# CyberAgentAILab/layout-dm

Measured on AMD Instinct MI355X. Metric: layouts/sec (whole node), Rico25 uncond T=100, higher is better.
Workload: dtype f16 (f32 accumulate); 1 GPU; BASELINE config 2: rico25 cond=unconditional T=100 batch=512/GPU sampling=random; precision_mode=fast, launch=one launch per sampling call (reverse loop resident in the layout's workgroup), chunk_layouts=256, lanes=2, parallelism=dp1 (independent layout shards, one all_gather of the final tokens)

## Files before the change

layout_dm_amd/csrc/kernels_stack.hip:

```cpp
#include <cstdlib>

#include "ldm_kernels.h"
#include "ldm_dma.h"
#include "ldm_pipes.h"
#include "ldm_post_dpp.h"
#include "ldm_relation_core.h"

namespace ldm {

struct StackArgs {
  FusedLayerSet ls;
  float* x;
  int ldx, N, S, H, n_chunks;
  float scale_log2e;
  const char* head_img;
  const float *head_g, *head_b;
  float* logits;
  int ldl, n_head_tiles;
  PostArgs post;
  const float* adaln;
  StackTables tbl;
  int32_t* inter;
  int n_steps, inter_ld, tie_ld;
  int16_t t_model[kStackLoopMaxSteps], t_post[kStackLoopMaxSteps];
// ... 2 lines not shown
};
typedef const __attribute__((address_space(4))) StackArgs* stack_kargs_ptr;
__device__ __forceinline__ stack_kargs_ptr stack_kargs() {
  stack_kargs_ptr q = (stack_kargs_ptr)__builtin_amdgcn_kernarg_segment_ptr();
  asm volatile("" : "+s"(q));
  return q;
}
constexpr int kPostLd = 161;
constexpr int kPostRows = 128 * kPostLd * 4;
constexpr int kStackLoopB1 = 2048;
constexpr int kStackLoopRelLds = REL_MAX_EDGE * 4 + 4 * 32 * 4 + 16;
constexpr int kStackLoopLds = 1024 + 128 + 2304;
static_assert(kRelIncBytes <= 2304, "incidence lists outgrow their LDS slot");
static_assert(kRelScratchFloats * 4 <= 2 * KV_BYTES, "the SGD's scratch lives in the K / V buffers");

__device__ unsigned long long g_stack_phase[16];

__device__ __forceinline__ int stack_lane_id() {
  int l;
  asm volatile("v_mbcnt_lo_u32_b32 %0, -1, 0\n\tv_mbcnt_hi_u32_b32 %0, -1, %0" : "=v"(l));
  return l;
}

__device__ __forceinline__ float stack_xor32_swap(float v) {
  const auto sw = __builtin_amdgcn_permlane32_swap(__float_as_uint(v), __float_as_uint(v), false, false);
  return (stack_lane_id() & 32) ? __uint_as_float(sw[0]) : __uint_as_float(sw[1]);
}
#define LDM_XOR32(v) (HEAD == 2 ? stack_xor32_swap(v) : __shfl_xor(v, 32, 64))

template <bool TM, int HEAD, bool REL = false>
__global__ __launch_bounds__(256, 1) void stack_stream_k(StackArgs a) {
  static_assert(!REL || HEAD == 2, "the relation tail belongs to the loop kernel");
  constexpr int KS = 29, STAGE = TILE_STAGE, NT2 = 15, NGV = 58;
  extern __shared__ __attribute__((aligned(16))) char smem[];
  const int tid_o = threadIdx.x;
  const int wave_o = __builtin_amdgcn_readfirstlane(tid_o >> 6);
  const int b_o = blockIdx.x;

  unsigned long long t0 = 0, t_real0 = 0, s_pro = 0, s_stream = 0, s_core = 0, s_slab = 0, s_ln2 = 0, s_ffn = 0, s_bnd = 0, s_bnd_a = 0, s_bnd_b = 0, s_hsync = 0, s_ssync = 0;
  if constexpr (TM) {
    t0 = __builtin_amdgcn_s_memtime();
    t_real0 = __builtin_amdgcn_s_memrealtime();
  }
  f32x16 acc[NT2];
  if constexpr (HEAD == 2) {
    const stack_kargs_ptr kp = stack_kargs();
    const int S = kp->S;
    int* toks = reinterpret_cast<int*>(smem + 3 * STAGE + 2 * KV_BYTES + (3 * kp->H * 64 + 2 * LN_DP + 512 + kStackLoopB1 + 2 * LN_DP + 512) * 4);
    if (tid_o < 128) {
      const int s = tid_o < S ? tid_o : S - 1;
      const size_t row = (size_t)b_o * S + s;
      toks[tid_o] = kp->post.tokens[row];
      int cc = -1;
      if (kp->post.cond_seq) cc = kp->post.cond_seq[row] | ((kp->post.strong && kp->post.strong[row]) ? (1 << 30) : 0);
      toks[128 + tid_o] = cc;
    }
    if constexpr (REL) {
      if (tid_o == 0) {
        int k = 1;
        const int A5 = kp->post.v.n_attr;
        for (int e = 0; e < S / A5; ++e)
          toks[256 + e] = ((kp->post.cond_seq[(size_t)b_o * S + e * A5]) != kp->post.v.pad_id) ? k++ : -1;
      }
      const int e0 = kp->rel.edge_off[b_o], ne = kp->rel.edge_off[b_o + 1] - e0;
      relation_incidence(kp->rel, e0, ne, tid_o, S / kp->post.v.n_attr, reinterpret_cast<float*>(smem + 3 * STAGE), toks + 288,
                         reinterpret_cast<unsigned short*>(toks + 288 + kRelIncOffInts), [] { __syncthreads(); });
// ... 61 lines not shown
      v2[k] = in ? w.b2[i] : 0.f;
    }
    __builtin_amdgcn_sched_barrier(0);
#pragma unroll
    for (int k = 0; k < 6; ++k) sbias[tid + 256 * k] = vb[k];
#pragma unroll
    for (int k = 0; k < 8; ++k)
      if (tid + 256 * k < A.n_chunks * 32) sb1[tid + 256 * k] = v1[k];
#pragma unroll
    for (int k = 0; k < 2; ++k) {
      const int i = tid + 256 * k;
      sp[i] = 1.0f + vs[k];
      sp[LN_DP + i] = vh[k];
      sbo[i] = vo[k] + vh[k];
      sp2[i] = vg[k];
      sp2[LN_DP + i] = ve[k];
      sb2[i] = v2[k];
    }
  };
  auto dma_table = [&](const float* g, const float* lds_dst, int n_kib) {
    const unsigned dst = lds0 + (unsigned)(reinterpret_cast<const char*>(lds_dst) - smem);
    for (int k = wave; k < n_kib; k += 4) {
      asm volatile("s_mov_b32 m0, %0\n\ts_nop 0" ::"s"(dst + k * 1024) : "memory");
      dma_lin<0>(voff, reinterpret_cast<const char*>(g) + (size_t)k * 1024);
    }
  };
  auto dma_first_tiles = [&](const char* img) {
#pragma unroll
    for (int k = 0; k < 4; ++k) dma_lin4(voff, img + wave * 8192 + (k >> 1) * STAGE + (k & 1) * 4096,
                                         lds0 + wave * 8192 + (k >> 1) * STAGE + (k & 1) * 4096);
  };
  int t_model = 0;
  if constexpr (HEAD == 2) t_model = stack_kargs()->t_model[it];
#pragma unroll
  for (int i = 8; i < 16; ++i) acc[NT2 - 1][i] = to_agpr(0.f);
  if constexpr (HEAD == 2) {
    const int lane = stack_lane_id();
    const int r = lane & 31, hi = lane >> 5;
    const int row = wave * 32 + r;
    const int srow = row < S ? row : S - 1;
    const stack_kargs_ptr kp = stack_kargs();
    dma_table(kp->tbl.att_static, sbias, kStackTblAttStatic / 256);
    dma_table(kp->tbl.att_dyn + (size_t)t_model * L * kStackTblAttDyn, sp, kStackTblAttDyn / 256);
    const float* erow = kp->post.emb + (size_t)toks[srow] * kp->post.D + hi * 4;
    const float* prow = kp->post.pos + (size_t)srow * kp->post.D + hi * 4;
    constexpr int GB = 12;
#pragma unroll
    for (int g0 = 0; g0 < NGV; g0 += GB) {
      float4 re[GB], rp[GB];
#pragma unroll
      for (int i = 0; i < GB; ++i)
        if (g0 + i < NGV) {
          re[i] = *reinterpret_cast<const float4*>(erow + (g0 + i) * 8);
          rp[i] = *reinterpret_cast<const float4*>(prow + (g0 + i) * 8);
        }
      __builtin_amdgcn_sched_barrier(0);
#pragma unroll
      for (int i = 0; i < GB; ++i) {
        const int gg = g0 + i;
        if (gg < NGV) {
          const int t = gg >> 2, q0 = (gg & 3) * 4;
          acc[t][q0 + 0] = to_agpr(re[i].x + rp[i].x);
          acc[t][q0 + 1] = to_agpr(re[i].y + rp[i].y);
          acc[t][q0 + 2] = to_agpr(re[i].z + rp[i].z);
          acc[t][q0 + 3] = to_agpr(re[i].w + rp[i].w);
        }
      }
      __builtin_amdgcn_sched_barrier(0);
    }
  } else {
    const int lane = stack_lane_id();
    const int r = lane & 31, hi = lane >> 5;
    const int row = wave * 32 + r;
    const size_t m = (size_t)b * S + (row < S ? row : S - 1);
    constexpr int GB = 20;
    const float* rrow = A.x + m * A.ldx + hi * 4;
#pragma unroll
    for (int g0 = 0; g0 < NGV; g0 += GB) {
      float4 raw[GB];
#pragma unroll
      for (int i = 0; i < GB; ++i)
        if (g0 + i < NGV) raw[i] = *reinterpret_cast<const float4*>(rrow + (g0 + i) * 8);
      __builtin_amdgcn_sched_barrier(0);
#pragma unroll
      for (int i = 0; i < GB; ++i) {
        const int gg = g0 + i;
        if (gg < NGV) {
          const int t = gg >> 2, q0 = (gg & 3) * 4;
          acc[t][q0 + 0] = to_agpr(raw[i].x);
          acc[t][q0 + 1] = to_agpr(raw[i].y);
          acc[t][q0 + 2] = to_agpr(raw[i].z);
          acc[t][q0 + 3] = to_agpr(raw[i].w);
        }
      }
      __builtin_amdgcn_sched_barrier(0);
    }
  }
  if constexpr (TM) s_pro = __builtin_amdgcn_s_memtime() - t0;

  for (int l = 0; l < L; ++l) {
    const auto& w = A.ls.w[l];
    unsigned long long tL = 0;
    if constexpr (TM) tL = __builtin_amdgcn_s_memtime();
    f16x8 xf[KS];
    {
      if constexpr (HEAD == 2) {
        asm volatile("s_waitcnt vmcnt(0)" ::: "memory");
        __builtin_amdgcn_s_barrier();
        asm volatile("" ::: "memory");
        dma_first_tiles((const char*)w.img);
        dma_table(stack_kargs()->tbl.ffn + (size_t)l * kStackTblFfn, sb1, kStackTblFfn / 256);
      } else {
        __builtin_amdgcn_s_barrier();
        asm volatile("" ::: "memory");
        dma_first_tiles((const char*)w.img);
        stage_tables(w, w.ada_scale, w.ada_shift, tid);
        __syncthreads();
      }
      unsigned long long tE1 = 0, tE2 = 0;
      if constexpr (TM) tE1 = __builtin_amdgcn_s_memtime();
      const int lane3 = stack_lane_id();
      const int hi3 = lane3 >> 5;
      float s1 = 0.f, s2 = 0.f;
#pragma unroll
      for (int t = 0; t < NT2; ++t) {
        const f32x16 tile = acc[t];
#pragma unroll
        for (int i = 0; i < 16; ++i)
          if (t * 4 + (i >> 2) < NGV) {
            s1 += tile[i];
            s2 += tile[i] * tile[i];
          }
        __builtin_amdgcn_sched_barrier(0);
      }
      s1 += LDM_XOR32(s1);
      s2 += LDM_XOR32(s2);
      if constexpr (TM) tE2 = __builtin_amdgcn_s_memtime();
      constexpr float kInvN3 = 1.0f / 464.0f;
      const float mean = s1 * kInvN3;
      const float rstd = 1.0f / sqrtf(fmaxf(s2 * kInvN3 - mean * mean, 0.f) + 1e-5f);
      const float ra = rstd, rb = -mean * rstd;
      const float* gmp = sp + hi3 * 4;
      const float* tbp = sbo + hi3 * 4;
#pragma unroll
      for (int t = 0; t < NT2; ++t) {
        f32x16 tile = acc[t];
#pragma unroll
        for (int g = 0; g < 4; ++g) {
          const int gg = t * 4 + g;
// ... 76 lines not shown
          AC.hi = hi;
          AC.run(nf);
        }
        if constexpr (TM) tC = __builtin_amdgcn_s_memtime();
        {
          const int lane = stack_lane_id();
          const int r = lane & 31, hi = lane >> 5;
          SlabPair<NT2, TM> SP;
          SP.acc = acc;
          SP.voff = voff;
          SP.lds_w = lds0 + wave * 8192;
          SP.aS[0] = lds0 + r * 64 + (((0 + hi) ^ ((r >> 2) & 3)) << 4);
          SP.aS[1] = lds0 + r * 64 + (((2 + hi) ^ ((r >> 2) & 3)) << 4);
          SP.nf = nf;
          SP.gnext = gimg + (size_t)8 * STAGE;
          SP.run();
          if constexpr (TM) s_ssync += SP.t_sync;
        }
        if constexpr (TM) {
          s_stream += tB - tA;
          s_core += tC - tB;
          s_slab += __builtin_amdgcn_s_memtime() - tC;
        }
      }
    }
    unsigned long long t_att = 0, t_ln2 = 0;
    if constexpr (TM) t_att = __builtin_amdgcn_s_memtime();
    asm volatile("s_waitcnt vmcnt(0) lgkmcnt(0)" ::: "memory");
    __builtin_amdgcn_s_barrier();
    asm volatile("" ::: "memory");
    {
      const char* g0 = (const char*)w.ffn_img + wave * 16384;
#pragma unroll
      for (int k = 0; k < 4; ++k) dma_lin4(voff, g0 + k * 4096, lds0 + wave * 16384 + k * 4096);
    }
    if constexpr (HEAD == 2) {
      const stack_kargs_ptr kp = stack_kargs();
      if (l + 1 < L) {
        dma_table(kp->tbl.att_static + (size_t)(l + 1) * kStackTblAttStatic, sbias, kStackTblAttStatic / 256);
        dma_table(kp->tbl.att_dyn + ((size_t)t_model * L + l + 1) * kStackTblAttDyn, sp, kStackTblAttDyn / 256);
      } else {
        dma_table(kp->tbl.head, sp, kStackTblAttDyn / 256);
      }
    }
    const int lane2 = stack_lane_id();
    const int r2 = lane2 & 31, hi2 = lane2 >> 5;
    f16x8 xf2[KS];
    {
      float s1 = 0.f, s2 = 0.f;
#pragma unroll
      for (int t = 0; t < NT2; ++t) {
        const f32x16 tile = acc[t];
#pragma unroll
        for (int i = 0; i < 16; ++i)
          if (t * 4 + (i >> 2) < NGV) {
            s1 += tile[i];
            s2 += tile[i] * tile[i];
          }
        __builtin_amdgcn_sched_barrier(0);
      }
      s1 += LDM_XOR32(s1);
      s2 += LDM_XOR32(s2);
      constexpr float kInvN = 1.0f / 464.0f;
      const float mean = s1 * kInvN;
      const float rstd = 1.0f / sqrtf(fmaxf(s2 * kInvN - mean * mean, 0.f) + 1e-5f);
      const float* gp = sp2 + hi2 * 4;
      const float* bp = sb2 + hi2 * 4;
#pragma unroll
      for (int t = 0; t < NT2; ++t) {
        f32x16 tile = acc[t];
#pragma unroll
        for (int g = 0; g < 4; ++g) {
          const int gg = t * 4 + g;
          if (gg < NGV) {
            const int ks = gg >> 1, e0 = (gg & 1) * 4;
            const float4 ga = *reinterpret_cast<const float4*>(gp + gg * 8);
            const float4 be = *reinterpret_cast<const float4*>(gp + LN_DP + gg * 8);
            const float4 bb = *reinterpret_cast<const float4*>(bp + gg * 8);
            const float v0 = tile[g * 4 + 0], v1 = tile[g * 4 + 1], v2 = tile[g * 4 + 2], v3 = tile[g * 4 + 3];
            xf2[ks][e0 + 0] = (_Float16)fmaf((v0 - mean) * rstd, ga.x, be.x);
            xf2[ks][e0 + 1] = (_Float16)fmaf((v1 - mean) * rstd, ga.y, be.y);
            xf2[ks][e0 + 2] = (_Float16)fmaf((v2 - mean) * rstd, ga.z, be.z);
            xf2[ks][e0 + 3] = (_Float16)fmaf((v3 - mean) * rstd, ga.w, be.w);
            tile[g * 4 + 0] = v0 + bb.x;
            tile[g * 4 + 1] = v1 + bb.y;
            tile[g * 4 + 2] = v2 + bb.z;
            tile[g * 4 + 3] = v3 + bb.w;
            if (gg & 1) asm volatile("" : "+v"(xf2[ks]));
          }
        }
        asm volatile("" : "+a"(tile));
        acc[t] = tile;
        __builtin_amdgcn_sched_barrier(0);
      }
    }
    if constexpr (TM) t_ln2 = __builtin_amdgcn_s_memtime();
    {
      unsigned relW1[8], relW2[2];
#pragma unroll
      for (int k = 0; k < 8; ++k) relW1[k] = r2 * RKB + ((((k << 1) | hi2) ^ (r2 & 15)) << 4);
#pragma unroll
      for (int sx = 0; sx < 2; ++sx) relW2[sx] = r2 * 64 + (((2 * sx + hi2) ^ ((r2 >> 2) & 3)) << 4);
      const unsigned relB = lds0 + (unsigned)(reinterpret_cast<char*>(sb1) - smem) + hi2 * 16;
      FfnStream<KS, NT2, 2, false, 6, true> F;
      F.xf = xf2;
      F.acc = acc;
      F.voff = voff;
      asm volatile("s_waitcnt vmcnt(0) lgkmcnt(0)" ::: "memory");
      __builtin_amdgcn_s_barrier();
      asm volatile("" ::: "memory");
#pragma unroll
      for (int k = 0; k < 8; ++k) F.aW1[k] = lds0 + relW1[k];
#pragma unroll
      for (int sx = 0; sx < 2; ++sx) F.aW2[sx] = lds0 + relW2[sx];
      F.ab_next = relB;
#pragma unroll
      for (int k = 0; k < KS; ++k) asm volatile("" : "+v"(xf2[k]));
      __builtin_amdgcn_s_waitcnt(0x0F70);
      __builtin_amdgcn_sched_barrier(0);
      F.read_bias();
      F.template prologue<0>();
      {
        const f16x8 z = {(_Float16)0.f, (_Float16)0.f, (_Float16)0.f, (_Float16)0.f,
                         (_Float16)0.f, (_Float16)0.f, (_Float16)0.f, (_Float16)0.f};
        F.pf[0] = F.pf[1] = F.pfn[0] = F.pfn[1] = z;
      }
      const char* fimg = (const char*)w.ffn_img;
      for (int c = 0; c <= A.n_chunks; ++c) {
#if !defined(LDM_ABL_FFN_WINDOW)
        F.gnext = fimg + (size_t)(c == A.n_chunks ? 0 : c + 1) * FFN_STAGE + wave * 16384;
#elif LDM_ABL_FFN_WINDOW == 1
        F.gnext = fimg + wave * 16384;
#else
        F.gnext = fimg;
#endif
        F.mnext = lds0 + ((c + 1) & 1) * FFN_STAGE + wave * 16384;
        F.ab_next = relB + (c + 1 >= A.n_chunks ? 0 : c + 1) * 128;
        F.template step<0, true>();
      }
      asm volatile("s_waitcnt vmcnt(0) lgkmcnt(0)" ::: "memory");
      __builtin_amdgcn_sched_barrier(0);
    }
    unsigned long long t_ffn = 0;
    if constexpr (TM) {
      t_ffn = __builtin_amdgcn_s_memtime();
      s_ln2 += t_ln2 - t_att;
      s_ffn += t_ffn - t_ln2;
    }
  }
  if constexpr (TM) t_epi = __builtin_amdgcn_s_memtime();
  {
    __builtin_amdgcn_s_barrier();
    asm volatile("" ::: "memory");
    auto dma_head_tile = [&](int ht) {
      const char* g = A.head_img + (size_t)ht * STAGE + wave * 8192;
      const unsigned l = lds0 + (unsigned)(ht & 3) * STAGE + wave * 8192;
      dma_lin4(voff, g, l);
      dma_lin4(voff, g + 4096, l + 4096);
    };
    for (int ht = 0; ht < 3 && ht < A.n_head_tiles; ++ht) dma_head_tile(ht);
    if constexpr (HEAD != 2) {
      for (int i = tid_now(); i < LN_DP; i += 256) {
        sp[i] = i < A.N ? A.head_g[i] : 0.f;
        sp[LN_DP + i] = i < A.N ? A.head_b[i] : 0.f;
      }
    }
    __syncthreads();
    const int lane3 = stack_lane_id();
    const int r3 = lane3 & 31, hi3 = lane3 >> 5;
    const int row3 = wave * 32 + r3;
    f16x8 xf3[KS];
// ... 18 lines not shown
      const float ra = rstd, rb = -mean * rstd;
      const float* gmp = sp + hi3 * 4;
#pragma unroll
      for (int t = 0; t < NT2; ++t) {
        const f32x16 tile = acc[t];
#pragma unroll
        for (int g = 0; g < 4; ++g) {
          const int gg = t * 4 + g;
          if (gg < NGV) {
            const int ks = gg >> 1, e0 = (gg & 1) * 4;
            const float4 gm = *reinterpret_cast<const float4*>(gmp + gg * 8);
            const float4 be = *reinterpret_cast<const float4*>(gmp + LN_DP + gg * 8);
            xf3[ks][e0 + 0] = (_Float16)fmaf(fmaf(tile[g * 4 + 0], ra, rb), gm.x, be.x);
            xf3[ks][e0 + 1] = (_Float16)fmaf(fmaf(tile[g * 4 + 1], ra, rb), gm.y, be.y);
            xf3[ks][e0 + 2] = (_Float16)fmaf(fmaf(tile[g * 4 + 2], ra, rb), gm.z, be.z);
            xf3[ks][e0 + 3] = (_Float16)fmaf(fmaf(tile[g * 4 + 3], ra, rb), gm.w, be.w);
            if (gg & 1) asm volatile("" : "+v"(xf3[ks]));
          }
        }
        __builtin_amdgcn_sched_barrier(0);
      }
    }
#pragma unroll
    for (int k = 0; k < KS; ++k) asm volatile("" : "+v"(xf3[k]));
    __builtin_amdgcn_s_waitcnt(0x0F70);
    __builtin_amdgcn_sched_barrier(0);
    const bool valid3 = row3 < S;
    float* lrow = HEAD == 2 ? nullptr : A.logits + ((size_t)b * S + (valid3 ? row3 : S - 1)) * A.ldl + hi3 * 4;
    unsigned relW[8];
#pragma unroll
    for (int k = 0; k < 8; ++k) relW[k] = lds0 + r3 * RKB + ((((k << 1) | hi3) ^ (r3 & 15)) << 4);
    if constexpr (HEAD == 2) {
      constexpr int NHT = 5;
#pragma unroll
      for (int ht = 0; ht < NHT; ++ht) {
        asm volatile("s_waitcnt vmcnt(0) lgkmcnt(0)" ::: "memory");
        __builtin_amdgcn_s_barrier();
        asm volatile("" ::: "memory");
        if (ht + 3 < NHT) dma_head_tile(ht + 3);
        TilePipe<KS, 8> TP;
        TP.xf = xf3;
        TP.voff = voff;
#pragma unroll
        for (int k = 0; k < 8; ++k) TP.aW[k] = relW[k] + (unsigned)(ht & 3) * STAGE;
        TP.template run<false, false>();
        f32x16 lg = TP.acc;
        asm volatile("s_nop 7\n\ts_nop 7" : "+v"(lg));
        asm volatile("" : "+a"(lg));
        acc[ht] = lg;
      }
      __builtin_amdgcn_s_barrier();
      asm volatile("" ::: "memory");
      const stack_kargs_ptr kp = stack_kargs();
      const auto& p = kp->post;
      float* lgs = reinterpret_cast<float*>(smem);
      float4* rstat = reinterpret_cast<float4*>(smem + kPostRows);
      float* ssch = reinterpret_cast<float*>(smem + kPostRows + 2048) + wave * 128;
      const int Cm1 = p.v.n_class - 1;
      const int t_post = kp->t_post[it];
      {
        float mx = -INFINITY, am = 0.f;
#pragma unroll
        for (int ht = 0; ht < NHT; ++ht) {
          const f32x16 tile = acc[ht];
#pragma unroll
          for (int i = 0; i < 16; ++i)
            if (ht * 32 + (i >> 2) * 8 + hi3 * 4 + (i & 3) < Cm1) {
              mx = fmaxf(mx, tile[i]);
              am = fmaxf(am, fabsf(tile[i]));
            }
        }
        mx = fmaxf(mx, LDM_XOR32(mx));
        am = fmaxf(am, LDM_XOR32(am));
        float se = 0.f;
        float* mine = lgs + row3 * kPostLd + hi3 * 4;
#pragma unroll
        for (int ht = 0; ht < NHT; ++ht) {
          const f32x16 tile = acc[ht];
#pragma unroll
          for (int i = 0; i < 16; ++i) {
            if (ht * 32 + (i >> 2) * 8 + hi3 * 4 + (i & 3) < Cm1) se += __expf(tile[i] - mx);
            mine[ht * 32 + (i >> 2) * 8 + (i & 3)] = tile[i];
          }
        }
        se += LDM_XOR32(se);
        if (hi3 == 0) rstat[row3] = make_float4(mx, __logf(se), am, 0.f);
        const int T1 = p.T + 1, u = (t_post - 1 + T1) % T1;
        if (lane3 < p.v.n_attr * 10) {
          const int at = lane3 / 10, k = lane3 - at * 10;
          const int kind = k == 0 ? kLogAt : k == 1 ? kLogBt : k == 2 ? kLogCt : k == 3 ? kLogCumAt : k == 4 ? kLogCumBt
                         : k == 5 ? kLogCumCt : k == 6 ? kLogCumAt : k == 7 ? kLogCumBt : k == 8 ? kLogCumCt : kLog1mCumCt;
          ssch[lane3] = p.sched[((size_t)kind * p.v.n_attr + at) * T1 + (k < 6 ? t_post : u)];
        }
        if (lane3 < p.v.n_attr) {
          reinterpret_cast<int*>(ssch)[100 + 2 * lane3] = p.v.start[lane3];
          reinterpret_cast<int*>(ssch)[101 + 2 * lane3] = p.v.count[lane3];
        }
      }
      __builtin_amdgcn_s_waitcnt(0xc07f);
      __builtin_amdgcn_wave_barrier();
      {
        const int lane5 = stack_lane_id();
        if (lane5 < 2 * p.v.n_attr) {
          const float* sc10 = ssch + (lane5 >> 1) * 10;
          const ldm_post::StepSchedule sc{sc10[0], sc10[1], sc10[2], sc10[3], sc10[4],
                                          sc10[5], sc10[6], sc10[7], sc10[8], sc10[9]};
          const ldm_post::QTerms k = ldm_post::q_terms(ldm_post::DppGroup<16, true>{0}, (lane5 & 1) != 0, sc);
          float* o = ssch + 50 + lane5 * 5;
          o[0] = k.qt_same; o[1] = k.qt_other; o[2] = k.q1_same; o[3] = k.q1_other; o[4] = k.q1_mask;
        }
      }
      __builtin_amdgcn_s_waitcnt(0xc07f);
      __builtin_amdgcn_wave_barrier();
      {
        const int lane4 = stack_lane_id();
        const int grp = lane4 >> 4;
        const ldm_post::DppGroup<16, true> g{lane4 & 15};
        const ldm_post::SlotMap<16, 3, true> m{lane4 & 15};
        const bool last = it + 1 == n_iter;
        bool adjust = false;
        if constexpr (REL) adjust = kp->t_model[it] >= 10 && kp->rel.num_update > 0;
        [[maybe_unused]] const int* node_of = condc + 128;
#pragma unroll 2
        for (int rd = 0; rd < 8; ++rd) {
          const int s = wave * 32 + rd * 4 + grp;
          if (s < S) {
            const int attr = s % p.v.n_attr;
            const float* sc10 = ssch + attr * 10;
            const ldm_post::StepSchedule sc{sc10[0], sc10[1], sc10[2], sc10[3], sc10[4],
                                            sc10[5], sc10[6], sc10[7], sc10[8], sc10[9]};
            const int cc = condc[s];
            ldm_post::TokenArgs ta{};
            ta.tok = toks[s];
            ta.start = reinterpret_cast<const int*>(ssch)[100 + 2 * attr];
            ta.count = reinterpret_cast<const int*>(ssch)[101 + 2 * attr];
            ta.pad_id = p.v.pad_id;
            ta.mask_id = p.v.mask_id;
            ta.n_class = p.v.n_class;
            ta.cond_tok = cc < 0 ? -1 : (cc & 0x3fffffff);
            ta.strong = cc >= 0 && (cc >> 30) != 0;
            ta.weak = p.weak ? p.weak + (size_t)b * p.v.n_class * S + s : nullptr;
            ta.weak_stride = S;
            ta.pad_disable = !adjust && p.pad_disable && cc >= 0 && attr != 0 && ta.cond_tok != p.v.pad_id;
            ta.kind = p.kind;
            ta.temperature = p.temperature;
            ta.top_p = p.top_p;
            ta.top_k = p.top_k;
            ta.pos = (uint32_t)s;
            ta.step = (uint32_t)(p.step + it);
            ta.layout = p.rng[1] + (uint64_t)p.layout_off + (uint64_t)b;
            ta.seed = p.rng[0];
            bool shortcut = ldm_post::strong_shortcut(ta);
            if constexpr (REL) shortcut = shortcut && !(adjust && attr != 0 && node_of[s / p.v.n_attr] > 0);
            if (shortcut) {
              if (g.lane() == 0) {
                toks[s] = ta.cond_tok;
                if (kp->inter) kp->inter[((size_t)it * kp->inter_ld + b) * S + s] = ta.cond_tok;
                if (last) p.tokens_out[(size_t)b * S + s] = ta.cond_tok;
              }
              continue;
            }
            float* lrow_s = lgs + s * kPostLd;
            const float4 rs = rstat[s];
            float l0[3], lp[3];
#pragma unroll
            for (int j = 0; j < 3; ++j) {
              const int c = m.cls(ta, j);
              l0[j] = (m.valid(ta, j) && c < Cm1) ? ldm_post::l0_f32(lrow_s[c], rs.x, rs.y) : -70.0f;
            }
            const float* qk = ssch + 50 + (attr * 2 + (ta.tok == ta.mask_id ? 1 : 0)) * 5;
            float k0 = qk[0], k1 = qk[1], k2 = qk[2], k3 = qk[3], k4 = qk[4];
            asm volatile("" : "+v"(k0), "+v"(k1), "+v"(k2), "+v"(k3), "+v"(k4));
            const ldm_post::QTerms k{k0, k1, k2, k3, k4};
            ldm_post::token_log_probs(g, m, ta, sc, k, l0, lp);
            if constexpr (REL) {
              if (adjust) {
#pragma unroll
                for (int j = 0; j < 3; ++j)
                  if (m.valid(ta, j)) lrow_s[m.sidx(j)] = lp[j];
                continue;
              }
            }
            const ldm_post::Draw d = ldm_post::draw_token(g, m, ta, lp, lrow_s, lrow_s + 48, false);
            if (g.lane() == 0) {
              toks[s] = d.token;
              if (kp->inter) kp->inter[((size_t)it * kp->inter_ld + b) * S + s] = d.token;
// ... 163 lines not shown
```

layout_dm_amd/csrc/ldm_dma.h:

```cpp
#pragma once
#include <hip/hip_runtime.h>

#include "ldm_kernels.h"

namespace ldm {

using dma_f16x8 = __attribute__((ext_vector_type(8))) _Float16;
constexpr int kLnDp = 512;

__device__ __forceinline__ void dma_set_m0(unsigned lds_addr) {
  asm volatile("s_mov_b32 m0, %0" ::"s"(lds_addr) : "memory");
}
template <int OFF>
__device__ __forceinline__ void dma_lin(unsigned voff, const char* sbase) {
  asm volatile("global_load_lds_dwordx4 %0, %1 offset:%2" ::"v"(voff), "s"(sbase), "n"(OFF) : "memory");
}
__device__ __forceinline__ void dma_lin4(unsigned voff, const char* sbase, unsigned lds_addr) {
  asm volatile(
      "s_mov_b32 m0, %2\n\ts_nop 0\n\t"
      "global_load_lds_dwordx4 %0, %1\n\t"
      "global_load_lds_dwordx4 %0, %1 offset:1024\n\t"
      "global_load_lds_dwordx4 %0, %1 offset:2048\n\t"
      "global_load_lds_dwordx4 %0, %1 offset:3072" ::"v"(voff),
      "s"(sbase), "s"(lds_addr)
      : "memory");
}

}
```

layout_dm_amd/csrc/ldm_loop.cpp:

```cpp
#include "ldm_handle.h"

using namespace ldm_host;

void ldm_host::fill_post(ldm_handle* h, PostArgs& p, const ldm_cond* cond, const ldm_sampler* s, size_t layout_off,
                      int Bc) {
  p.sched = h->sched;
  p.f32_lse = h->cfg.precision == LDM_PREC_FAST_F16 ? 1 : 0;
  p.T = h->T;
  p.B = Bc;
  p.S = h->S;
  p.v = h->vocab;
  p.rng = h->rng;
  if (cond) {
    const size_t ro = layout_off * h->S;
    p.cond_seq = cond->d_cond_seq ? cond->d_cond_seq + ro : nullptr;
    p.strong = cond->d_strong_mask ? cond->d_strong_mask + ro : nullptr;
    p.weak = cond->d_weak_logits ? cond->d_weak_logits + layout_off * h->C * h->S : nullptr;
    p.pad_disable = cond->pad_disable;
  }
  if (s) {
    p.kind = s->kind;
    p.temperature = s->temperature;
    p.top_p = s->top_p;
    p.top_k = s->top_k;
// ... 123 lines not shown
      a.logp_tm = 1;
      a.cond_seq = cond->d_cond_seq + (size_t)off * h->S;
      fill_rel(h, a, rel, rel_layout_off + off, Bc);
      ldm_handle::Scope sc(h, st, "relation_update", 0, (double)Bc * 4 * h->cfg.n_bin * h->cfg.max_elem * 8);
      launch_relation_update(a, st);
    }
    {
      PostArgs q{};
      fill_post(h, q, cond, s, off, Bc);
      q.strong = nullptr;
      q.weak = nullptr;
      q.pad_disable = 1;
      q.logp_in = ws.rel_logp;
      q.logp_tm = 1;
      q.tokens_out = tout + (size_t)off * h->S;
      q.step = step;
      q.layout_off = (int)(rng_layout_off + off);
      if (embed_next) {
        q.x_next = ws.P; q.emb = h->emb; q.pos = h->pos; q.D = h->D; q.ldx = h->D;
      }
      ldm_handle::Scope sc(h, st, "pad_disable_sample", 0, (double)Bc * h->S * (h->C * 4 + 8));
      launch_posterior_sample(q, st);
    }
  }
  return 0;
}

bool ldm_host::loop_fusable(const ldm_handle* h, const ldm_relation* rel) {
  int live_max = 0;
  for (int a = 0; a < h->cfg.n_attr; ++a) live_max = std::max(live_max, h->vocab.count[a] + 2);
  if (rel && (h->rel_loop == 0 || h->cfg.q_type != LDM_Q_CONSTRAINED || h->cfg.n_bin > 32 || h->cfg.max_elem > 32 ||
              h->cfg.n_attr != 5))
    return false;
  return h->stack_loop && h->cfg.precision == LDM_PREC_FAST_F16 && h->fused_attn == 6 && h->head_img_ks && h->Cp == 160 && live_max <= kStackPostMaxLive && h->S <= 128 &&
         h->T < 32768 && !h->fast.empty() && h->tbl_att_dyn && h->D == 464 && h->F <= 2048;
}

static int run_loop_fused(ldm_handle* h, const int32_t* tin, int32_t* tout, const ldm_cond* cond, const ldm_relation* rel,
                          const int32_t* t_model, const int32_t* t_post, int n_steps, const ldm_sampler* s, int step0, int B,
                          int32_t* d_inter, int tie_row0, hipStream_t st) {
  const int D = h->D, F = h->F, M = B * h->S;
  FusedLayerSet ls{};
  ls.n_layer = h->L;
  for (int i = 0; i < h->L; ++i) {
    const LayerW& w = h->layers[i];
    ls.w[i] = FusedLayerW{h->fast[i].attn_head_img_ks, h->fast[i].b_in, nullptr, nullptr, h->fast[i].b_out_v,
                          h->fast[i].ffn_img_pipe, w.b1, w.b2, w.g2, w.be2};
  }
  const StackHead hd{h->head_img_ks, h->head_g, h->head_b, nullptr, h->Cp, h->Cp / 32};
  const double step_flops = h->L * (gemm_flops(M, 3 * D, D) + 4.0 * B * h->H * (double)h->S * h->S * h->dh +
                                    gemm_flops(M, D, D) + 2 * gemm_flops(M, F, D)) + gemm_flops(M, h->C, D);
  for (int i0 = 0; i0 < n_steps; i0 += kStackLoopMaxSteps) {
    const int n = std::min(kStackLoopMaxSteps, n_steps - i0);
    PostArgs p{};
    fill_post(h, p, cond, s, 0, B);
    p.tokens = i0 == 0 ? tin : tout;
    p.tokens_out = tout;
    p.step = step0 + i0;
    p.layout_off = 0;
    p.emb = h->emb; p.pos = h->pos; p.D = D;
    RelArgs ra{};
    if (rel) {
      p.pad_disable = 1;
      fill_rel(h, ra, rel, 0, B);
    }
    if (tie_row0 >= 0 && h->tie_rel > 0.f && h->tie_flags && s->kind == LDM_SAMPLE_DETERMINISTIC) {
      p.tie_flags = h->tie_flags + (size_t)(tie_row0 + i0) * h->cfg.max_batch;
// ... 265 lines not shown
```

layout_dm_amd/csrc/ldm_pipes.h:

```cpp
#pragma once
#include <hip/hip_runtime.h>
#include <hip/hip_fp16.h>

#include "ldm_dma.h"
#include "ldm_kernels.h"
#include "ldm_stream_sched.h"

namespace ldm {

using f32x16 = __attribute__((ext_vector_type(16))) float;
using f16x8 = __attribute__((ext_vector_type(8))) _Float16;

constexpr int RK = 512;
constexpr int RKB = RK * 2;
constexpr int W1_STAGE = 32 * RKB;
constexpr int TILE_STAGE = 32 * RKB;
constexpr int FFN_STAGE = 65536;
constexpr int LN_DP = 512;
constexpr int KV_BYTES = 128 * 128;

typedef __attribute__((address_space(3))) char* lds_char_ptr;

template <int OFF>
__device__ __forceinline__ void dsr128(f16x8& d, unsigned addr) {
// ... 77 lines not shown
                   : __builtin_amdgcn_mfma_f32_32x32x16_f16(cur, xf[IT], acc, 0, 0, 0);
      }
      __builtin_amdgcn_sched_barrier(0);
      if constexpr (IT + PF < KS) read_item<IT + PF>();
      if constexpr (DMA && IT % 2 == 1) dma_slot<IT / 2>();
      else if constexpr (DMA) dma_m0<IT / 2>();
      step<IT + 1, SWAP, DMA>();
    }
  }
  template <int IT>
  __device__ __forceinline__ void prologue() {
    if constexpr (IT < PF) {
      read_item<IT>();
      prologue<IT + 1>();
    }
  }
  template <bool SWAP, bool DMA = true>
  __device__ __forceinline__ void run() {
    prologue<0>();
    step<0, SWAP, DMA>();
  }
};

template <int S8>
__device__ __forceinline__ f16x8 cvt8(const f32x16& a, const float4& b0, const float4& b1) {
  f16x8 o;
  o[0] = (_Float16)(a[S8 + 0] + b0.x); o[1] = (_Float16)(a[S8 + 1] + b0.y);
  o[2] = (_Float16)(a[S8 + 2] + b0.z); o[3] = (_Float16)(a[S8 + 3] + b0.w);
  o[4] = (_Float16)(a[S8 + 4] + b1.x); o[5] = (_Float16)(a[S8 + 5] + b1.y);
  o[6] = (_Float16)(a[S8 + 6] + b1.z); o[7] = (_Float16)(a[S8 + 7] + b1.w);
  return o;
}

template <int KS, int NT2, int DE, bool TM, int PFQ = 6, bool PIPE = false>
struct FfnStream {
  using SCH = ldm_sched::FfnSched<KS, NT2, PFQ>;
  static constexpr int PF = SCH::PF;
  static constexpr int NIT = SCH::NIT;
  static constexpr int SYNC = SCH::SYNC;
  unsigned long long tA, tB, tC, tD, t_sync = 0;
  f16x8 q[PF];
  unsigned aW1[8], aW2[2];
  const f16x8* xf;
  f32x16 ha, hb;
  f32x16* acc;
  f16x8 pf[2], pfn[2];
  float4 bb[4];
  static constexpr int IPW = 16;
  const char* gnext;
  unsigned mnext, voff, ab_next;

  template <int J>
  __device__ __forceinline__ void dma_m0() {
    if constexpr (J < IPW && (J & 3) == 0) dma_set_m0(mnext + (J >> 2) * 4096);
  }
  template <int J>
  __device__ __forceinline__ void dma_slot() {
    if constexpr (J < IPW) dma_lin<(J & 3) * 1024>(voff, gnext + (J >> 2) * 4096);
  }
  template <int IT>
  __device__ __forceinline__ void read_item() {
    constexpr int I = IT % NIT;
    if constexpr (I < KS) {
      dsr128<256 * (I >> 3)>(q[IT % PF], aW1[I & 7]);
    } else if constexpr (I == KS) {
      dsr128<0>(q[IT % PF], aW1[0]);
    } else {
      constexpr int sx = (I - KS - 1) / NT2, t = (I - KS - 1) % NT2;
      dsr128<W1_STAGE + t * 2048>(q[IT % PF], aW2[sx]);
    }
  }
  __device__ __forceinline__ void read_bias() {
    dsr128f<0>(bb[0], ab_next);
    dsr128f<32>(bb[1], ab_next);
    dsr128f<64>(bb[2], ab_next);
    dsr128f<96>(bb[3], ab_next);
  }
  template <int IT, bool DMA>
  __device__ __forceinline__ void step() {
    if constexpr (IT < NIT) {
      wait_lgkm<SCH::after(IT)>();
      __builtin_amdgcn_sched_barrier(0);
      const f16x8 cur = q[IT % PF];
      if constexpr (IT == 0) {
        f32x16 bv;
#pragma unroll
        for (int rq = 0; rq < 4; ++rq) {
          bv[rq * 4 + 0] = bb[rq].x; bv[rq * 4 + 1] = bb[rq].y; bv[rq * 4 + 2] = bb[rq].z; bv[rq * 4 + 3] = bb[rq].w;
        }
        asm volatile("v_mfma_f32_32x32x16_f16 %0, %1, %2, %3" : "=&v"(ha) : "v"(cur), "v"(xf[0]), "v"(bv));
      } else if constexpr (IT == 1) {
        asm volatile("v_mfma_f32_32x32x16_f16 %0, %1, %2, 0" : "=&v"(hb) : "v"(cur), "v"(xf[1]));
      } else if constexpr (IT < KS) {
        if constexpr (IT % 2 == 0) asm volatile("v_mfma_f32_32x32x16_f16 %0, %1, %2, %0" : "+v"(ha) : "v"(cur), "v"(xf[IT]));
        else asm volatile("v_mfma_f32_32x32x16_f16 %0, %1, %2, %0" : "+v"(hb) : "v"(cur), "v"(xf[IT]));
        if constexpr (IT == KS - 1 && !PIPE) asm volatile("s_nop 15" ::: "memory");
      } else if constexpr (IT == KS && PIPE) {
        (void)cur;
      } else if constexpr (IT == KS) {
        (void)cur;
        typedef __attribute__((ext_vector_type(2))) float f32x2v;
        typedef __attribute__((ext_vector_type(2))) _Float16 f16x2v;
#pragma unroll
        for (int i = 0; i < 8; ++i) {
          const f32x2v sa = {ha[2 * i], ha[2 * i + 1]}, sb = {hb[2 * i], hb[2 * i + 1]};
          const f16x2v hv = __builtin_convertvector(sa + sb, f16x2v);
          const f16x2v zero = {(_Float16)0.f, (_Float16)0.f};
          const f16x2v r = __builtin_elementwise_max(hv, zero);
          pf[i >> 2][(i & 3) * 2 + 0] = r[0];
          pf[i >> 2][(i & 3) * 2 + 1] = r[1];
        }
      } else {
        constexpr int sx = (IT - KS - 1) / NT2, t = (IT - KS - 1) % NT2;
        acc[t] = __builtin_amdgcn_mfma_f32_32x32x16_f16(cur, pf[sx], acc[t], 0, 0, 0);
        if constexpr (PIPE) {
          constexpr int g = IT - KS - 1;
          if constexpr (g >= 2 && g < 10) {
            constexpr int i = g - 2;
            typedef __attribute__((ext_vector_type(2))) _Float16 f16x2v;
            const float s0 = ha[2 * i] + hb[2 * i], s1 = ha[2 * i + 1] + hb[2 * i + 1];
            f16x2v hv = {(_Float16)s0, (_Float16)s1};
            const f16x2v zero = {(_Float16)0.f, (_Float16)0.f};
            hv = __builtin_elementwise_max(hv, zero);
            pfn[i >> 2][(i & 3) * 2 + 0] = hv[0];
            pfn[i >> 2][(i & 3) * 2 + 1] = hv[1];
          }
        }
      }
      if constexpr (PIPE && IT == 0) {
        pf[0] = pfn[0];
        pf[1] = pfn[1];
      }
      __builtin_amdgcn_sched_barrier(0);
      if constexpr (TM && IT == KS - 1) tC = __builtin_amdgcn_s_memtime();
      if constexpr (TM && IT == KS + 1) tD = __builtin_amdgcn_s_memtime();
      if constexpr (IT == SYNC) {
        if constexpr (TM) tA = __builtin_amdgcn_s_memtime();
        asm volatile("s_waitcnt vmcnt(0)" ::: "memory");
        __builtin_amdgcn_s_barrier();
        asm volatile("" ::: "memory");
        if constexpr (TM) {
          tB = __builtin_amdgcn_s_memtime();
          t_sync += tB - tA;
        }
        read_bias();
#pragma unroll
        for (int sx = 0; sx < 2; ++sx) aW2[sx] ^= 0x10000u;
      }
      read_item<IT + PF>();
      if constexpr (IT == KS - 1 - PF) {
#pragma unroll
        for (int k = 0; k < 8; ++k) aW1[k] ^= 0x10000u;
      }
      if constexpr (DMA && IT % DE == DE - 1) dma_slot<IT / DE>();
      else if constexpr (DMA && IT % DE == 0) dma_m0<IT / DE>();
      step<IT + 1, DMA>();
    }
  }
  template <int IT>
  __device__ __forceinline__ void prologue() {
    if constexpr (IT < PF) {
      read_item<IT>();
      prologue<IT + 1>();
    }
  }
};

template <bool TM = false, bool LEAN = false>
struct HeadStream {
  using SCH = ldm_sched::HeadSched<LEAN>;
  static constexpr int KS = SCH::KS, NT = SCH::NT, NIT = SCH::NIT, PF = SCH::PF, SYNC = SCH::SYNC, EPI0 = SCH::EPI0;
  static_assert(NT % 3 == 0, "ring stage of a tile is a compile-time constant");
  f16x8 q[PF];
  unsigned aW[8], aW2[8];
  const f16x8* xf;
  f32x16 accA, accB;
  float4 bb[4];
  f16x8* qf;
  unsigned aK[2], aV[2];
  unsigned a_bias;
  const char* gimg;
  unsigned lds_w;
  unsigned voff;
  int h, H;
  unsigned long long t_sync = 0;

  static constexpr bool tile_has_bias(int j) { return SCH::tile_has_bias(j); }
  static constexpr int younger(int G) { return SCH::younger(G); }

// ... 279 lines not shown
```

layout_dm_amd/csrc/ldm_stream_sched.h:

```cpp
#pragma once

namespace ldm_sched {

template <bool LEAN>
struct HeadSched {
  static constexpr int KS = 29, NT = 6, NIT = KS * NT, PF = 6;
  static constexpr int SYNC = KS - PF;
  static constexpr int EPI0 = 10;
  static constexpr int BIAS_LEAN = EPI0 - PF - 1;

  static constexpr bool tile_has_bias(int j) { return j < 2 || j >= 4; }
  static constexpr int bias_at(int s) {
    const int j = s / KS, it = s % KS;
    if (LEAN) return ((it == BIAS_LEAN && j >= 1 && tile_has_bias(j - 1)) || (j == NT - 1 && it == SYNC)) ? 4 : 0;
    return (it == SYNC && j + 1 < NT && tile_has_bias(j + 1)) ? 4 : 0;
  }
  static constexpr int writes_at(int s) {
    const int j = s / KS, it = s % KS;
    return (j >= 1 && j <= 4 && (it == EPI0 + 2 || it == EPI0 + 5)) ? 1 : 0;
  }
  static constexpr int prologue_bias() { return LEAN ? 0 : 4; }
  static constexpr int younger(int G) {
    int cnt = 0;
    bool seen = false;
    for (int i = 0; i < PF; ++i) {
      if (seen) ++cnt;
      if (i == G) seen = true;
    }
    for (int s = 0; s < G; ++s) {
      if (seen) cnt += bias_at(s);
      if (s + PF < NIT) {
        if (seen) ++cnt;
        if (s + PF == G) seen = true;
      }
      if (seen) cnt += writes_at(s);
    }
    return cnt;
  }
};

template <int KS, int NT2, int PFQ>
struct FfnSched {
  static constexpr int PF = PFQ, NIT = KS + 1 + 2 * NT2, SYNC = NIT - PF;
  static_assert(NIT % PF == 0, "queue slots must line up across chunks");
  static_assert(PF - 1 + 4 <= 15, "lgkmcnt is a 4-bit counter");
  static constexpr int after(int IT) { return IT > SYNC ? PF - 1 + 4 : PF - 1; }
};

}
```

Before: 3795 layouts/s.

## Interleave FFN double-buffer ring so stage lives in ds_read immediates

Reorganizes the FFN weight ring in LDS so the two stages of each half sit side by side, letting the stage be encoded in the ds_read immediate offset. The chunk loop is unrolled by two with the stage as a template argument, which removes the per-chunk address XOR toggles and the pf/pfn register copy. It also builds accumulator tiles whole with padding zeros instead of a separate zeroing loop, and hardcodes five attributes in the post step. A new gate requiring C-1 > 128 keeps the simplified head masking valid, at the cost of more code size and reliance on fixed config assumptions.

```diff
diff --git a/layout_dm_amd/csrc/kernels_stack.hip b/layout_dm_amd/csrc/kernels_stack.hip
--- a/layout_dm_amd/csrc/kernels_stack.hip
+++ b/layout_dm_amd/csrc/kernels_stack.hip
@@ -58,6 +58,7 @@
 __global__ __launch_bounds__(256, 1) void stack_stream_k(StackArgs a) {
   static_assert(!REL || HEAD == 2, "the relation tail belongs to the loop kernel");
   constexpr int KS = 29, STAGE = TILE_STAGE, NT2 = 15, NGV = 58;
+  using FfnRing = ldm_sched::FfnRingInterleaved;
   extern __shared__ __attribute__((aligned(16))) char smem[];
   const int tid_o = threadIdx.x;
   const int wave_o = __builtin_amdgcn_readfirstlane(tid_o >> 6);
@@ -185,8 +186,7 @@
   };
   int t_model = 0;
   if constexpr (HEAD == 2) t_model = stack_kargs()->t_model[it];
-#pragma unroll
-  for (int i = 8; i < 16; ++i) acc[NT2 - 1][i] = to_agpr(0.f);
+  static_assert(NGV == 4 * NT2 - 2, "columns 464..479 (the last two groups of tile NT2 - 1) are padding: zero, written with the gather");
   if constexpr (HEAD == 2) {
     const int lane = stack_lane_id();
     const int r = lane & 31, hi = lane >> 5;
@@ -209,14 +209,21 @@
         }
       __builtin_amdgcn_sched_barrier(0);
 #pragma unroll
-      for (int i = 0; i < GB; ++i) {
-        const int gg = g0 + i;
-        if (gg < NGV) {
-          const int t = gg >> 2, q0 = (gg & 3) * 4;
-          acc[t][q0 + 0] = to_agpr(re[i].x + rp[i].x);
-          acc[t][q0 + 1] = to_agpr(re[i].y + rp[i].y);
-          acc[t][q0 + 2] = to_agpr(re[i].z + rp[i].z);
-          acc[t][q0 + 3] = to_agpr(re[i].w + rp[i].w);
+      for (int tb = 0; tb < GB / 4; ++tb) {
+        const int t = g0 / 4 + tb;
+        if (t < NT2) {
+          f32x16 tile;
+#pragma unroll
+          for (int g = 0; g < 4; ++g) {
+            const int i = tb * 4 + g;
+            const bool in = t * 4 + g < NGV;
+            tile[g * 4 + 0] = in ? re[i].x + rp[i].x : 0.f;
+            tile[g * 4 + 1] = in ? re[i].y + rp[i].y : 0.f;
+            tile[g * 4 + 2] = in ? re[i].z + rp[i].z : 0.f;
+            tile[g * 4 + 3] = in ? re[i].w + rp[i].w : 0.f;
+          }
+          asm volatile("" : "+a"(tile));
+          acc[t] = tile;
         }
       }
       __builtin_amdgcn_sched_barrier(0);
@@ -236,14 +243,21 @@
         if (g0 + i < NGV) raw[i] = *reinterpret_cast<const float4*>(rrow + (g0 + i) * 8);
       __builtin_amdgcn_sched_barrier(0);
 #pragma unroll
-      for (int i = 0; i < GB; ++i) {
-        const int gg = g0 + i;
-        if (gg < NGV) {
-          const int t = gg >> 2, q0 = (gg & 3) * 4;
-          acc[t][q0 + 0] = to_agpr(raw[i].x);
-          acc[t][q0 + 1] = to_agpr(raw[i].y);
-          acc[t][q0 + 2] = to_agpr(raw[i].z);
-          acc[t][q0 + 3] = to_agpr(raw[i].w);
+      for (int tb = 0; tb < GB / 4; ++tb) {
+        const int t = g0 / 4 + tb;
+        if (t < NT2) {
+          f32x16 tile;
+#pragma unroll
+          for (int g = 0; g < 4; ++g) {
+            const int i = tb * 4 + g;
+            const bool in = t * 4 + g < NGV;
+            tile[g * 4 + 0] = in ? raw[i].x : 0.f;
+            tile[g * 4 + 1] = in ? raw[i].y : 0.f;
+            tile[g * 4 + 2] = in ? raw[i].z : 0.f;
+            tile[g * 4 + 3] = in ? raw[i].w : 0.f;
+          }
+          asm volatile("" : "+a"(tile));
+          acc[t] = tile;
         }
       }
       __builtin_amdgcn_sched_barrier(0);
@@ -267,7 +281,9 @@
         __builtin_amdgcn_s_barrier();
         asm volatile("" ::: "memory");
         dma_first_tiles((const char*)w.img);
-        stage_tables(w, w.ada_scale, w.ada_shift, tid);
+        int tid_l = tid;
+        asm volatile("" : "+v"(tid_l));
+        stage_tables(w, w.ada_scale, w.ada_shift, tid_l);
         __syncthreads();
       }
       unsigned long long tE1 = 0, tE2 = 0;
@@ -410,7 +426,7 @@
     {
       const char* g0 = (const char*)w.ffn_img + wave * 16384;
 #pragma unroll
-      for (int k = 0; k < 4; ++k) dma_lin4(voff, g0 + k * 4096, lds0 + wave * 16384 + k * 4096);
+      for (int k = 0; k < 4; ++k) dma_lin4(voff, g0 + k * 4096, lds0 + FfnRing::dma_dst(0, wave, 0) + k * 4096);
     }
     if constexpr (HEAD == 2) {
       const stack_kargs_ptr kp = stack_kargs();
@@ -476,11 +492,11 @@
     {
       unsigned relW1[8], relW2[2];
 #pragma unroll
-      for (int k = 0; k < 8; ++k) relW1[k] = r2 * RKB + ((((k << 1) | hi2) ^ (r2 & 15)) << 4);
-#pragma unroll
-      for (int sx = 0; sx < 2; ++sx) relW2[sx] = r2 * 64 + (((2 * sx + hi2) ^ ((r2 >> 2) & 3)) << 4);
+      for (int k = 0; k < 8; ++k) relW1[k] = ldm_sched::ffn_w1_lane(r2, hi2, k);
+#pragma unroll
+      for (int sx = 0; sx < 2; ++sx) relW2[sx] = ldm_sched::ffn_w2_lane(r2, hi2, sx);
       const unsigned relB = lds0 + (unsigned)(reinterpret_cast<char*>(sb1) - smem) + hi2 * 16;
-      FfnStream<KS, NT2, 2, false, 6, true> F;
+      FfnStream<KS, NT2, 2, false, 6, true, FfnRing> F;
       F.xf = xf2;
       F.acc = acc;
       F.voff = voff;
@@ -490,7 +506,7 @@
 #pragma unroll
       for (int k = 0; k < 8; ++k) F.aW1[k] = lds0 + relW1[k];
 #pragma unroll
-      for (int sx = 0; sx < 2; ++sx) F.aW2[sx] = lds0 + relW2[sx];
+      for (int sx = 0; sx < 2; ++sx) F.aW2[sx] = lds0 + FfnRing::w2(0) + relW2[sx];
       F.ab_next = relB;
 #pragma unroll
       for (int k = 0; k < KS; ++k) asm volatile("" : "+v"(xf2[k]));
@@ -504,7 +520,8 @@
         F.pf[0] = F.pf[1] = F.pfn[0] = F.pfn[1] = z;
       }
       const char* fimg = (const char*)w.ffn_img;
-      for (int c = 0; c <= A.n_chunks; ++c) {
+      F.mnext = lds0 + FfnRing::dma_dst(0, wave, 0);
+      auto chunk_args = [&](int c) {
 #if !defined(LDM_ABL_FFN_WINDOW)
         F.gnext = fimg + (size_t)(c == A.n_chunks ? 0 : c + 1) * FFN_STAGE + wave * 16384;
 #elif LDM_ABL_FFN_WINDOW == 1
@@ -512,9 +529,18 @@
 #else
         F.gnext = fimg;
 #endif
-        F.mnext = lds0 + ((c + 1) & 1) * FFN_STAGE + wave * 16384;
         F.ab_next = relB + (c + 1 >= A.n_chunks ? 0 : c + 1) * 128;
-        F.template step<0, true>();
+      };
+      int c = 0;
+      for (; c + 1 <= A.n_chunks; c += 2) {
+        chunk_args(c);
+        F.template step<0, true, 0>();
+        chunk_args(c + 1);
+        F.template step<0, true, 1>();
+      }
+      if (c <= A.n_chunks) {
+        chunk_args(c);
+        F.template step<0, true, 0>();
       }
       asm volatile("s_waitcnt vmcnt(0) lgkmcnt(0)" ::: "memory");
       __builtin_amdgcn_sched_barrier(0);
@@ -599,6 +625,7 @@
     for (int k = 0; k < 8; ++k) relW[k] = lds0 + r3 * RKB + ((((k << 1) | hi3) ^ (r3 & 15)) << 4);
     if constexpr (HEAD == 2) {
       constexpr int NHT = 5;
+      constexpr int NA = 5;
 #pragma unroll
       for (int ht = 0; ht < NHT; ++ht) {
         asm volatile("s_waitcnt vmcnt(0) lgkmcnt(0)" ::: "memory");
@@ -632,7 +659,7 @@
           const f32x16 tile = acc[ht];
 #pragma unroll
           for (int i = 0; i < 16; ++i)
-            if (ht * 32 + (i >> 2) * 8 + hi3 * 4 + (i & 3) < Cm1) {
+            if (ht < NHT - 1 || ht * 32 + (i >> 2) * 8 + hi3 * 4 + (i & 3) < Cm1) {
               mx = fmaxf(mx, tile[i]);
               am = fmaxf(am, fabsf(tile[i]));
             }
@@ -646,20 +673,20 @@
           const f32x16 tile = acc[ht];
 #pragma unroll
           for (int i = 0; i < 16; ++i) {
-            if (ht * 32 + (i >> 2) * 8 + hi3 * 4 + (i & 3) < Cm1) se += __expf(tile[i] - mx);
+            if (ht < NHT - 1 || ht * 32 + (i >> 2) * 8 + hi3 * 4 + (i & 3) < Cm1) se += __expf(tile[i] - mx);
             mine[ht * 32 + (i >> 2) * 8 + (i & 3)] = tile[i];
           }
         }
         se += LDM_XOR32(se);
         if (hi3 == 0) rstat[row3] = make_float4(mx, __logf(se), am, 0.f);
         const int T1 = p.T + 1, u = (t_post - 1 + T1) % T1;
-        if (lane3 < p.v.n_attr * 10) {
+        if (lane3 < NA * 10) {
           const int at = lane3 / 10, k = lane3 - at * 10;
           const int kind = k == 0 ? kLogAt : k == 1 ? kLogBt : k == 2 ? kLogCt : k == 3 ? kLogCumAt : k == 4 ? kLogCumBt
                          : k == 5 ? kLogCumCt : k == 6 ? kLogCumAt : k == 7 ? kLogCumBt : k == 8 ? kLogCumCt : kLog1mCumCt;
-          ssch[lane3] = p.sched[((size_t)kind * p.v.n_attr + at) * T1 + (k < 6 ? t_post : u)];
-        }
-        if (lane3 < p.v.n_attr) {
+          ssch[lane3] = p.sched[((size_t)kind * NA + at) * T1 + (k < 6 ? t_post : u)];
+        }
+        if (lane3 < NA) {
           reinterpret_cast<int*>(ssch)[100 + 2 * lane3] = p.v.start[lane3];
           reinterpret_cast<int*>(ssch)[101 + 2 * lane3] = p.v.count[lane3];
         }
@@ -668,7 +695,7 @@
       __builtin_amdgcn_wave_barrier();
       {
         const int lane5 = stack_lane_id();
-        if (lane5 < 2 * p.v.n_attr) {
+        if (lane5 < 2 * NA) {
           const float* sc10 = ssch + (lane5 >> 1) * 10;
           const ldm_post::StepSchedule sc{sc10[0], sc10[1], sc10[2], sc10[3], sc10[4],
                                           sc10[5], sc10[6], sc10[7], sc10[8], sc10[9]};
@@ -692,7 +719,7 @@
         for (int rd = 0; rd < 8; ++rd) {
           const int s = wave * 32 + rd * 4 + grp;
           if (s < S) {
-            const int attr = s % p.v.n_attr;
+            const int attr = s % NA;
             const float* sc10 = ssch + attr * 10;
             const ldm_post::StepSchedule sc{sc10[0], sc10[1], sc10[2], sc10[3], sc10[4],
                                             sc10[5], sc10[6], sc10[7], sc10[8], sc10[9]};
@@ -718,7 +745,7 @@
             ta.layout = p.rng[1] + (uint64_t)p.layout_off + (uint64_t)b;
             ta.seed = p.rng[0];
             bool shortcut = ldm_post::strong_shortcut(ta);
-            if constexpr (REL) shortcut = shortcut && !(adjust && attr != 0 && node_of[s / p.v.n_attr] > 0);
+            if constexpr (REL) shortcut = shortcut && !(adjust && attr != 0 && node_of[s / NA] > 0);
             if (shortcut) {
               if (g.lane() == 0) {
                 toks[s] = ta.cond_tok;
diff --git a/layout_dm_amd/csrc/ldm_dma.h b/layout_dm_amd/csrc/ldm_dma.h
--- a/layout_dm_amd/csrc/ldm_dma.h
+++ b/layout_dm_amd/csrc/ldm_dma.h
@@ -10,6 +10,10 @@
 
 __device__ __forceinline__ void dma_set_m0(unsigned lds_addr) {
   asm volatile("s_mov_b32 m0, %0" ::"s"(lds_addr) : "memory");
+}
+template <unsigned OFF>
+__device__ __forceinline__ void dma_set_m0_add(unsigned lds_addr) {
+  asm volatile("s_add_u32 m0, %0, %1" ::"s"(lds_addr), "n"(OFF) : "memory", "scc");
 }
 template <int OFF>
 __device__ __forceinline__ void dma_lin(unsigned voff, const char* sbase) {
diff --git a/layout_dm_amd/csrc/ldm_loop.cpp b/layout_dm_amd/csrc/ldm_loop.cpp
--- a/layout_dm_amd/csrc/ldm_loop.cpp
+++ b/layout_dm_amd/csrc/ldm_loop.cpp
@@ -179,7 +179,7 @@
   if (rel && (h->rel_loop == 0 || h->cfg.q_type != LDM_Q_CONSTRAINED || h->cfg.n_bin > 32 || h->cfg.max_elem > 32 ||
               h->cfg.n_attr != 5))
     return false;
-  return h->stack_loop && h->cfg.precision == LDM_PREC_FAST_F16 && h->fused_attn == 6 && h->head_img_ks && h->Cp == 160 && live_max <= kStackPostMaxLive && h->S <= 128 &&
+  return h->stack_loop && h->cfg.precision == LDM_PREC_FAST_F16 && h->fused_attn == 6 && h->head_img_ks && h->Cp == 160 && h->C - 1 > 128 && live_max <= kStackPostMaxLive && h->S <= 128 &&
          h->T < 32768 && !h->fast.empty() && h->tbl_att_dyn && h->D == 464 && h->F <= 2048;
 }
 
diff --git a/layout_dm_amd/csrc/ldm_pipes.h b/layout_dm_amd/csrc/ldm_pipes.h
--- a/layout_dm_amd/csrc/ldm_pipes.h
+++ b/layout_dm_amd/csrc/ldm_pipes.h
@@ -133,7 +133,7 @@
   return o;
 }
 
-template <int KS, int NT2, int DE, bool TM, int PFQ = 6, bool PIPE = false>
+template <int KS, int NT2, int DE, bool TM, int PFQ = 6, bool PIPE = false, class MAP = ldm_sched::FfnRingLinear>
 struct FfnStream {
   using SCH = ldm_sched::FfnSched<KS, NT2, PFQ>;
   static constexpr int PF = SCH::PF;
@@ -151,18 +151,28 @@
   const char* gnext;
   unsigned mnext, voff, ab_next;
 
-  template <int J>
+  template <int J, int ST>
   __device__ __forceinline__ void dma_m0() {
-    if constexpr (J < IPW && (J & 3) == 0) dma_set_m0(mnext + (J >> 2) * 4096);
+    if constexpr (J < IPW && (J & 3) == 0) {
+      if constexpr (MAP::kStageInImm) dma_set_m0_add<MAP::dma_dst(ST ^ 1, 0, 0) + (J >> 2) * 4096>(mnext);
+      else dma_set_m0(mnext + (J >> 2) * 4096);
+    }
   }
   template <int J>
   __device__ __forceinline__ void dma_slot() {
     if constexpr (J < IPW) dma_lin<(J & 3) * 1024>(voff, gnext + (J >> 2) * 4096);
   }
-  template <int IT>
+  template <int IT, int ST = 0>
   __device__ __forceinline__ void read_item() {
     constexpr int I = IT % NIT;
-    if constexpr (I < KS) {
+    if constexpr (MAP::kStageInImm) {
+      constexpr int s = IT >= NIT ? (ST ^ 1) : ST;
+      constexpr unsigned off = MAP::template imm<KS, NT2>(I, s);
+      static_assert(off < 65536u, "ds_read offset field");
+      if constexpr (I < KS) dsr128<off>(q[IT % PF], aW1[I & 7]);
+      else if constexpr (I == KS) dsr128<off>(q[IT % PF], aW1[0]);
+      else dsr128<off>(q[IT % PF], aW2[(I - KS - 1) / NT2]);
+    } else if constexpr (I < KS) {
       dsr128<256 * (I >> 3)>(q[IT % PF], aW1[I & 7]);
     } else if constexpr (I == KS) {
       dsr128<0>(q[IT % PF], aW1[0]);
@@ -177,8 +187,12 @@
     dsr128f<64>(bb[2], ab_next);
     dsr128f<96>(bb[3], ab_next);
   }
-  template <int IT, bool DMA>
+  template <int IT, bool DMA, int ST = 0>
   __device__ __forceinline__ void step() {
+    static_assert(ST == 0 || MAP::kStageInImm, "the stage is a compile-time argument only where the map encodes it in the immediate");
+    constexpr bool SWP = PIPE && MAP::kStageInImm && ST == 1;
+    f16x8(&pcur)[2] = SWP ? pfn : pf;
+    [[maybe_unused]] f16x8(&pnew)[2] = SWP ? pf : pfn;
     if constexpr (IT < NIT) {
       wait_lgkm<SCH::after(IT)>();
       __builtin_amdgcn_sched_barrier(0);
@@ -213,7 +227,7 @@
         }
       } else {
         constexpr int sx = (IT - KS - 1) / NT2, t = (IT - KS - 1) % NT2;
-        acc[t] = __builtin_amdgcn_mfma_f32_32x32x16_f16(cur, pf[sx], acc[t], 0, 0, 0);
+        acc[t] = __builtin_amdgcn_mfma_f32_32x32x16_f16(cur, pcur[sx], acc[t], 0, 0, 0);
         if constexpr (PIPE) {
           constexpr int g = IT - KS - 1;
           if constexpr (g >= 2 && g < 10) {
@@ -223,12 +237,12 @@
             f16x2v hv = {(_Float16)s0, (_Float16)s1};
             const f16x2v zero = {(_Float16)0.f, (_Float16)0.f};
             hv = __builtin_elementwise_max(hv, zero);
-            pfn[i >> 2][(i & 3) * 2 + 0] = hv[0];
-            pfn[i >> 2][(i & 3) * 2 + 1] = hv[1];
+            pnew[i >> 2][(i & 3) * 2 + 0] = hv[0];
+            pnew[i >> 2][(i & 3) * 2 + 1] = hv[1];
           }
         }
       }
-      if constexpr (PIPE && IT == 0) {
+      if constexpr (PIPE && IT == 0 && !MAP::kStageInImm) {
         pf[0] = pfn[0];
         pf[1] = pfn[1];
       }
@@ -245,17 +259,19 @@
           t_sync += tB - tA;
         }
         read_bias();
-#pragma unroll
-        for (int sx = 0; sx < 2; ++sx) aW2[sx] ^= 0x10000u;
-      }
-      read_item<IT + PF>();
-      if constexpr (IT == KS - 1 - PF) {
+        if constexpr (!MAP::kStageInImm) {
+#pragma unroll
+          for (int sx = 0; sx < 2; ++sx) aW2[sx] ^= 0x10000u;
+        }
+      }
+      read_item<IT + PF, ST>();
+      if constexpr (IT == KS - 1 - PF && !MAP::kStageInImm) {
 #pragma unroll
         for (int k = 0; k < 8; ++k) aW1[k] ^= 0x10000u;
       }
       if constexpr (DMA && IT % DE == DE - 1) dma_slot<IT / DE>();
-      else if constexpr (DMA && IT % DE == 0) dma_m0<IT / DE>();
-      step<IT + 1, DMA>();
+      else if constexpr (DMA && IT % DE == 0) dma_m0<IT / DE, ST>();
+      step<IT + 1, DMA, ST>();
     }
   }
   template <int IT>
diff --git a/layout_dm_amd/csrc/ldm_stream_sched.h b/layout_dm_amd/csrc/ldm_stream_sched.h
--- a/layout_dm_amd/csrc/ldm_stream_sched.h
+++ b/layout_dm_amd/csrc/ldm_stream_sched.h
@@ -47,4 +47,35 @@
   static constexpr int after(int IT) { return IT > SYNC ? PF - 1 + 4 : PF - 1; }
 };
 
+constexpr unsigned ffn_w1_lane(int r, int hi, int k) { return (unsigned)(r * 1024 + ((((k << 1) | hi) ^ (r & 15)) << 4)); }
+constexpr unsigned ffn_w2_lane(int r, int hi, int sx) { return (unsigned)(r * 64 + (((2 * sx + hi) ^ ((r >> 2) & 3)) << 4)); }
+struct FfnRingLinear {
+  static constexpr bool kStageInImm = false;
+  static constexpr unsigned kHalf = 0x8000u, kRing = 0x20000u;
+  static constexpr unsigned w1(int s) { return (unsigned)s * 0x10000u; }
+  static constexpr unsigned w2(int s) { return (unsigned)s * 0x10000u + kHalf; }
+  static constexpr unsigned dma_dst(int s, int w, int k) { return (unsigned)s * 0x10000u + (unsigned)w * 0x4000u + (unsigned)k * 1024u; }
+  template <int KS, int NT2>
+  static constexpr unsigned reg_base(int) { return 0u; }
+  template <int KS, int NT2>
+  static constexpr unsigned imm(int I, int s) {
+    return (unsigned)s * 0x10000u + (I < KS ? 256u * (unsigned)(I >> 3) : I == KS ? 0u : kHalf + (unsigned)((I - KS - 1) % NT2) * 2048u);
+  }
+};
+struct FfnRingInterleaved {
+  static constexpr bool kStageInImm = true;
+  static constexpr unsigned kHalf = 0x8000u, kRing = 0x20000u;
+  static constexpr unsigned w1(int s) { return (unsigned)s * kHalf; }
+  static constexpr unsigned w2(int s) { return 0x10000u + (unsigned)s * kHalf; }
+  static constexpr unsigned dma_dst(int s, int w, int k) {
+    return (unsigned)(w >> 1) * 0x10000u + (unsigned)s * kHalf + (unsigned)(w & 1) * 0x4000u + (unsigned)k * 1024u;
+  }
+  template <int KS, int NT2>
+  static constexpr unsigned reg_base(int I) { return I <= KS ? 0u : 0x10000u; }
+  template <int KS, int NT2>
+  static constexpr unsigned imm(int I, int s) {
+    return (unsigned)s * kHalf + (I < KS ? 256u * (unsigned)(I >> 3) : I == KS ? 0u : (unsigned)((I - KS - 1) % NT2) * 2048u);
+  }
+};
+
 }
```

Result: faster. 3853 layouts/s (median of 6 runs) (+1.5%).
